# bioinformatics-centre/BayesTyper

Measured on AMD Instinct MI355X. Metric: variant-cluster Gibbs iterations/sec + k-mer matches/sec at 1/2/4/8 MI355X, higher is better.
Workload: dtype f64 log-probabilities over u8 k-mer counts (Gibbs); u64/u8 integer (k-mer matching)

## Files before the change

bayestyper_amd/csrc/bt_gibbs_simple.hpp:

```cpp
#pragma once
#include "bt_gibbs_tile.hpp"

namespace bt {

template <typename T>
struct LdsArr {
    T BT_LAS *p;
    __device__ inline T BT_LAS &operator[](uint32_t i) const { return p[i * LANES]; }
    __device__ inline LdsArr<T> operator+(uint32_t i) const { return LdsArr<T>{p + i * LANES}; }
};
template <typename T>
__device__ inline LdsArr<T> lds_arr(const Tile &t, int arr) {
    return LdsArr<T>{(T BT_LAS *)(bt_lds_raw + t.d->hoff[arr]) + t.lane};
}

struct Set2 {
    uint32_t n, e0, e1;
    __device__ inline void clear() { n = 0; }
    __device__ inline void insert(uint32_t e) {
        e1 = e0;
        e0 = e;
        ++n;
    }
    __device__ inline void erase(uint32_t e) {
// ... 232 lines not shown
        if (pv && pr > 255u) {
            log_collected_run(c, P, s, sd_key(pcode), pr, sc[SC_NSUB_U]);
            pr = 0;
            pv = 0;
        }
        blk[SB_WORDS * s + 2] = sd_code(dip[2 * s], dip[2 * s + 1]) | (pcode << SP_PDIP) | (wmax << SP_WMAX) | (pr << SP_PEND) | ((uint32_t)evn[s] << SP_EVN) | (pl << SP_PLOIDY) |
                                ((upd[s] ? 1u : 0u) << SP_UPD) | ((pv ? 1u : 0u) << SP_PVALID);
    }
    double p1 = 1.0;
    if (sc[SC_IS_SPARSE] && n_obs > 0) {
        TPtr<double> vec = c.simplex();
        const bool cached = d.scache_n && n_obs <= 2 * d.S && 1u <= d.scache_p;
        const uint32_t ci = cached ? (n_obs - 1) * d.scache_p : 0u;
        if (cached) vec = c.scache() + ci * d.scache_len;
        uint32_t len = cached ? (uint32_t)c.sclen()[ci] : 0u;
        if (len == 0) {
            len = simplex_prob_vector(c, P, vec, n_obs, 1u);
            if (cached) c.sclen()[ci] = len;
        }
        p1 = vec[0];
    }
    return p1;
}

__device__ static __noinline__ void simple_leave(Env env, uint32_t blk_off, double f0, double f1, uint32_t nzmask) {
    const Tile t = make_tile(env);
    const Vx c = make_vx(t, 0);
    const GParams BT_CAS &P = env_params(env);
    LdsArr<uint32_t> blk{(uint32_t BT_LAS *)(bt_lds_raw + blk_off) + t.lane};
    SPtrF<uint16_t, LANES> dip = c.dip(), pdip = c.pend_dip();
    SPtrF<uint32_t, LANES> pend = c.pend();
    SPtrF<uint8_t, LANES> pvalid = c.pend_valid(), upd = c.ksc_upd(), evn = c.evn();
    for (uint32_t s = 0; s < P.S; ++s) {
        const uint32_t pk = blk[SB_WORDS * s + 2];
        const uint32_t code = pk & 7u, pcode = (pk >> SP_PDIP) & 7u;
        dip[2 * s] = (uint16_t)sd_h1(code);
        dip[2 * s + 1] = (uint16_t)sd_h2(code);
        pdip[2 * s] = (uint16_t)sd_h1(pcode);
        pdip[2 * s + 1] = (uint16_t)sd_h2(pcode);
        pend[s] = (pk >> SP_PEND) & 255u;
        evn[s] = (uint8_t)((pk >> SP_EVN) & 255u);
        upd[s] = (uint8_t)((pk >> SP_UPD) & 1u);
        pvalid[s] = (uint8_t)((pk >> SP_PVALID) & 1u);
    }
    SPtrF<double, LANES> freq = c.freq(), logf = c.logf();
    SPtrF<uint8_t, LANES> nz = c.nz();
    freq[0] = f0;
    freq[1] = f1;
    nz[0] = (uint8_t)(nzmask & 1u);
    nz[1] = (uint8_t)((nzmask >> 1) & 1u);
    if (nzmask & 1u) logf[0] = bt_log(f0);
    if (nzmask & 2u) logf[1] = bt_log(f1);
}

__device__ static __noinline__ void simple_reweight(Env env, uint32_t blk_off) {
    const Tile t = make_tile(env);
    const Vx c = make_vx(t, 0);
    const GParams BT_CAS &P = env_params(env);
    simple_fill_unique(env);
    c.sc()[SC_UC_DIRTY] = 0;
    LdsArr<uint32_t> blk{(uint32_t BT_LAS *)(bt_lds_raw + blk_off) + t.lane};
    const Vx::UCPtr uc = c.ucache();
    const uint32_t Dcm = t.d->Dcm;
    for (uint32_t s = 0; s < P.S; ++s) {
        const uint32_t pk = blk[SB_WORDS * s + 2];
        const SimpleWeights w = simple_weights(uc, Dcm, s, (pk >> SP_PLOIDY) & 3u);
        blk[SB_WORDS * s] = __float_as_uint(w.ea);
        blk[SB_WORDS * s + 1] = __float_as_uint(w.eb);
        blk[SB_WORDS * s + 2] = (pk & ~(3u << SP_WMAX)) | (w.wmax << SP_WMAX);
    }
}
__device__ static __noinline__ void simple_noise_tally(Env env, uint32_t blk_off, const NoiseChainCtl *nc) {
    const Tile t = make_tile(env);
    const Vx c = make_vx(t, 0);
    const GParams BT_CAS &P = env_params(env);
    LdsArr<uint32_t> blk{(uint32_t BT_LAS *)(bt_lds_raw + blk_off) + t.lane};
    auto *bins = nc_bins(nc);
    const uint32_t nsu = c.sc()[SC_NSUB_U], Hm = t.d->Hm, S = P.S;
    const Vx::RPtr<uint8_t> sm = c.subm();
    TPtr<uint8_t> scn = c.subcnt(), sic = c.subic();
    for (uint32_t i = 0; i < nsu; i += 4) {
        uint8_t m0[4], m1[4], ic0[4], ic1[4];
#pragma unroll
        for (uint32_t r = 0; r < 4; ++r) {
            const uint32_t j = i + r < nsu ? i + r : nsu - 1u;
            m0[r] = sm[j * Hm];
            m1[r] = sm[j * Hm + 1];
            ic0[r] = sic[2 * j];
            ic1[r] = sic[2 * j + 1];
        }
        for (uint32_t s0 = 0; s0 < S; s0 += 4) {
            uint8_t cn[4][4];
#pragma unroll
            for (uint32_t w = 0; w < 4; ++w) {
                const uint32_t s = s0 + w < S ? s0 + w : S - 1u;
#pragma unroll
                for (uint32_t r = 0; r < 4; ++r) cn[w][r] = scn[(i + r < nsu ? i + r : nsu - 1u) * S + s];
            }
#pragma unroll
            for (uint32_t w = 0; w < 4; ++w) {
                const uint32_t s = s0 + w;
                if (s >= S) continue;
                const uint32_t code = blk[SB_WORDS * s + 2] & 7u, h1 = sd_h1(code), h2 = sd_h2(code);
                const bool g1 = P.gender[s] != 0;
#pragma unroll
                for (uint32_t r = 0; r < 4; ++r) {
                    uint8_t m = 0;
                    if (h1 != (uint32_t)NOHAP) m = (uint8_t)(m + (h1 ? m1[r] : m0[r]));
                    if (h2 != (uint32_t)NOHAP) m = (uint8_t)(m + (h2 ? m1[r] : m0[r]));
                    m = (uint8_t)(m + (g1 ? ic1[r] : ic0[r]));
                    if (i + r < nsu && m == 0) nc_tally(nc, bins, s, cn[w][r]);
                }
            }
        }
    }
    c.sc()[SC_UC_DIRTY] = 1;
}

__device__ inline void simple_sweeps(const Env &env, const Tile &t, const GParams BT_CAS &P, uint32_t n_burn, uint32_t n_collect, uint32_t *trace_counter, uint32_t *trace_buf,
                                     uint32_t trace_max, uint32_t tile, const NoiseChainCtl *nc = nullptr) {
    const uint32_t n_sweeps = n_burn + n_collect;
    const TileDesc BT_CAS &d = *t.d;
    const Vx c = make_vx(t, 0);
    const uint32_t S = P.S;
    const uint32_t blk_off = d.sblk;
    const double p_simplex1 = simple_enter(env, blk_off);
    LdsArr<uint32_t> blk{(uint32_t BT_LAS *)(bt_lds_raw + blk_off) + t.lane};
    SPtrF<uint32_t, LANES> sc = c.sc();
    const bool is_sparse = sc[SC_IS_SPARSE] != 0;
    Set2 zero{0, 0, 0}, plus{0, 0, 0};
    if (is_sparse) {
        zero = set2_load(c.zero_set());
        plus = set2_load(c.plus_set());
    }
    double fnd_saved = c.fnd_saved();
    uint32_t fnd_avail = sc[SC_FND_AVAIL];
    double f0, f1;
    uint32_t nzmask, obs0, obs1;
    {
        SPtrF<double, LANES> freq = c.freq();
        SPtrF<uint8_t, LANES> nz = c.nz();
        SPtrF<uint32_t, LANES> obs = c.obs();
        nzmask = (nz[0] ? 1u : 0u) | (nz[1] ? 2u : 0u);
        f0 = (nzmask & 1u) ? (double)freq[0] : 0.0;
        f1 = (nzmask & 2u) ? (double)freq[1] : 0.0;
        obs0 = obs[0];
        obs1 = obs[1];
    }
    typedef MtRingT<LdsArr<uint32_t>> Ring;
    const LdsArr<uint32_t> ring0 = lds_arr<uint32_t>(t, A_RING), ring1 = ring0 + (d.ring_cap[0] + MT_RING_HDR);
    Ring r0 = mt_ring_open_as(c.mt(0), ring0, d.ring_cap[0]), r1 = mt_ring_open_as(c.mt(1), ring1, d.ring_cap[1]);
    const double BT_GAS *a2tab = P.gamma_a2;
    const uint32_t a2n = P.gamma_n;

    const uint32_t sweep0 = nc ? nc->it_begin : 0u;
    for (uint32_t sweep = sweep0; sweep < n_sweeps; ++sweep) {
        const bool collect = sweep >= n_burn;
        if (nc && sweep > sweep0) {
            if (!nc_wait_table(nc, sweep)) break;
            if (nc->help_units) noise_help(env, nc);
            simple_reweight(env, blk_off);
        }
        bool tracing = false;
        TPtr<uint32_t> trace_row{(uint32_t BT_GAS *)trace_buf, 0u, 6u};
        if (trace_max) {
            uint32_t *cnt = &trace_counter[(size_t)tile * LANES + t.lane];
            const uint32_t n = *cnt;
            if (n < trace_max) {
                *cnt = n + 1;
                trace_row.off = (uint32_t)(d.trace_base + (size_t)n * d.nvm * S * LANES) + t.lane;
                tracing = true;
            }
        }
        PROF_DECL;
        {
            const uint32_t want = 2u * S < r0.cap - 3u ? 2u * S : r0.cap - 3u;
            if (bt_wave_any(r0.avail < want)) r0.topup();
            r1.topup();
        }
        PROF(11);
        const double ff00 = f0 * f0, ff01 = 2.0 * f0 * f1, ff11 = f1 * f1;
        const bool tiny = ((nzmask & 1u) && f0 < 1e-12) || ((nzmask & 2u) && f1 < 1e-12);
        for (uint32_t s = 0; s < S; ++s) {
            uint32_t pk = blk[SB_WORDS * s + 2];
            const float wa = __uint_as_float(blk[SB_WORDS * s]), wb = __uint_as_float(blk[SB_WORDS * s + 1]);
            const double u01 = rng_canonical(r0);
            const uint32_t pl = (pk >> SP_PLOIDY) & 3u, wmax = (pk >> SP_WMAX) & 3u, pcode = pk & 7u;
            uint32_t code = SD_NONE;
            if (pl != 0) {
                const double e0 = wmax == 0 ? 1.0 : (double)wa, e1 = wmax == 0 ? (double)wa : (wmax == 1 ? 1.0 : (double)wb), e2 = wmax == 2 ? 1.0 : (double)wb;
                const double w0 = (pl == 2 ? ff00 : f0) * e0, w1 = (pl == 2 ? ff01 : f1) * e1, w2 = pl == 2 ? ff11 * e2 : 0.0;
                const double c1 = w0 + w1, tot = c1 + w2, thr = u01 * tot, mg = 1e-5 * tot;
                const uint32_t pick = thr < w0 ? 0u : (thr < c1 ? 1u : 2u);
                const double lo = pick == 1 ? w0 : c1, hi = pick == 0 ? w0 : (pick == 1 ? c1 : tot);
                const bool safe = !tiny && tot > 1e-280 && hi - thr > mg && (pick == 0 || thr - lo > mg);
                code = pl == 2 ? pick : 3u + pick;
                if (!safe) {
                    PROF_CNT(19, 1);
                    code = simple_exact_code(env, s, pl, nzmask, f0, f1, u01);
                }
            }
            {
                const uint32_t h1 = sd_h1(code), h2 = sd_h2(code);
#pragma unroll
                for (uint32_t w = 0; w < 2; ++w) {
                    const uint32_t h = w ? h2 : h1;
                    if (h == (uint32_t)NOHAP) continue;
                    const uint32_t o = h ? obs1 : obs0;
                    if (is_sparse && o == 0) {
                        zero.erase(h);
                        plus.insert(h);
                    }
                    if (h) obs1 = o + 1;
                    else obs0 = o + 1;
                }
            }
            pk = (pk & ~7u) | code;
            if (code != pcode) pk |= 1u << SP_UPD;
            if (tracing) trace_row[s] = sd_key(code);
            if (collect) {
                const uint32_t pdc = (pk >> SP_PDIP) & 7u, run = (pk >> SP_PEND) & 255u;
                const bool pv = (pk >> SP_PVALID) & 1u;
                if (pv && pdc == code && run < 255u) pk += 1u << SP_PEND;
                else {
                    if (pv && run) {
                        uint32_t n = (pk >> SP_EVN) & 255u;
                        if (n == EV_CAP) {
                            simple_apply_full_log(env, s);
                            n = 0;
                        }
                        TPtr<uint32_t> lg = c.evlog(s);
                        lg[1 + 2 * n] = sd_key(pdc);
                        lg[2 + 2 * n] = run;
                        pk = (pk & ~(255u << SP_EVN)) | ((n + 1u) << SP_EVN);
                    }
                    pk = (pk & ~((7u << SP_PDIP) | (255u << SP_PEND))) | (code << SP_PDIP) | (1u << SP_PEND) | (1u << SP_PVALID);
                }
            }
            blk[SB_WORDS * s + 2] = pk;
        }
        PROF(2);
        const uint32_t n_obs = obs0 + obs1;
        if (n_obs > 0) {
            double saved = fnd_saved;
            uint32_t avail = fnd_avail;
            const NormalState nd{&saved, &avail};
            double g0 = 0, g1 = 0, norm = 0;
            bool sel0 = !is_sparse, sel1 = !is_sparse;
            uint32_t n_first = 2, n_steps = 2;
            Set2 order0 = plus;
            if (is_sparse) {
                const double u = rng_canonical(r1);
                n_first = plus.n;
                n_steps = plus.n + ((plus.n == 1 && !(u < p_simplex1)) ? 1u : 0u);
            }
            for (uint32_t i = 0; bt_wave_any(i < n_steps); ++i) {
                PROF_CNT(20, 1);
                if (i < n_steps) {
                    uint32_t e, o = 0;
                    if (!is_sparse) e = i;
                    else if (i < n_first) e = order0.at(i);
                    else {
                        const uint32_t pos = rng_uniform_int(r1, zero.n);
                        e = zero.at(pos);
                        zero.erase(e);
                        plus.insert(e);
                    }
                    if (i < n_first) o = e ? obs1 : obs0;
                    const uint32_t ai = o + 1u;
                    const double alpha = (double)ai, a1 = alpha - 1.0 / 3.0;
                    const double a2 = ai < a2n ? (double)a2tab[ai] : 1.0 / sqrt(9.0 * a1);
                    const double v = rng_gamma_v(r1, nd, a1, a2);
                    const double x = a1 * v * 1.0;
                    if (e) g1 = x, sel1 = true;
                    else g0 = x, sel0 = true;
                    norm += x;
                }
            }
            f0 = sel0 ? g0 / norm : 0.0;
            f1 = sel1 ? g1 / norm : 0.0;
            nzmask = (sel0 ? 1u : 0u) | (sel1 ? 2u : 0u);
            if (is_sparse) {
                const Set2 order = plus;
                plus.clear();
                for (uint32_t i = 0; i < 2; ++i)
                    if (i < order.n) zero.insert(order.at(i));
            }
            obs0 = obs1 = 0;
            fnd_saved = saved;
            fnd_avail = avail;
        }
        PROF(7);
        if (nc) {
            simple_noise_tally(env, blk_off, nc);
            if (!nc_iteration_end(nc, sweep)) break;
        }
    }
    mt_close(r0);
    mt_close(r1);
    if (is_sparse) {
        set2_store(c.zero_set(), zero);
        set2_store(c.plus_set(), plus);
    }
    c.fnd_saved() = fnd_saved;
    sc[SC_FND_AVAIL] = fnd_avail;
    sc[SC_HAP_COUNT] = obs0 + obs1;
// ... 11 lines not shown
```

bayestyper_amd/csrc/bt_gibbs_simple_kernel.hip:

```cpp
#define BT_SIMPLE_TU 1
#include "bt_gibbs_kernel.hpp"

namespace {
using namespace bt;
#ifndef GIBBS_SIMPLE_WAVES
#define GIBBS_SIMPLE_WAVES 3
#endif
__global__ __launch_bounds__(LANES, GIBBS_SIMPLE_WAVES) void gibbs_simple_kernel(const TileDesc *__restrict__ tiles, uint8_t *__restrict__ pool, const GParams *__restrict__ Pg,
                                                                                  int op, uint32_t arg0, uint32_t arg1, unsigned long long *__restrict__ hist, TraceCfg tr,
                                                                                  const uint32_t *__restrict__ tile_list) {
    gibbs_body<true>(tiles, pool, Pg, op, arg0, arg1, hist, tr, tile_list);
}
}

namespace bt {
hipError_t launch_gibbs_simple_kernel(unsigned grid, uint32_t lds, hipStream_t st, const TileDesc *tiles, uint8_t *pool, const GParams *P, int op, uint32_t a0, uint32_t a1,
                                      unsigned long long *hist, TraceCfg tr, const uint32_t *tile_list) {
    hipLaunchKernelGGL(gibbs_simple_kernel, dim3(grid), dim3(LANES), lds, st, tiles, pool, P, op, a0, a1, hist, tr, tile_list);
    return hipGetLastError();
}
#ifdef BT_PROF
hipError_t simple_prof_read(unsigned long long *h_out32, int reset) {
    hipError_t e = hipMemcpyFromSymbol(h_out32, HIP_SYMBOL(g_bt_prof), 32 * 8);
    if (e == hipSuccess && reset) {
        unsigned long long z[32] = {0};
        e = hipMemcpyToSymbol(HIP_SYMBOL(g_bt_prof), z, 32 * 8);
    }
    return e;
}
#endif
hipError_t prepare_gibbs_simple_kernel(int max_lds) {
    return hipFuncSetAttribute(reinterpret_cast<const void *>(gibbs_simple_kernel), hipFuncAttributeMaxDynamicSharedMemorySize, max_lds);
}
}
```

bayestyper_amd/csrc/bt_gibbs_tile.hpp:

```cpp
#pragma once
#include "bt_rng_device.hpp"

namespace bt {

constexpr unsigned LANES = 64;
constexpr uint16_t NOHAP = 0xFFFF;
constexpr double BT_LN2 = 0.693147180559945309417232121458176568;
constexpr double BT_DBL_EPS = 2.220446049250313080847263336181640625e-16;
#ifndef BT_LINEAR_DRAW_MIN
#define BT_LINEAR_DRAW_MIN 4u
#endif
#ifndef BT_UC_INVALIDATE_MIN
#define BT_UC_INVALIDATE_MIN 64u
#endif
#ifndef BT_EVAL_BLOCK
#define BT_EVAL_BLOCK 4u
#endif
constexpr uint32_t EVB = BT_EVAL_BLOCK;
#ifdef BT_SINGLE
constexpr bool kSingle = true;
#else
constexpr bool kSingle = false;
#endif
#ifdef BT_PACKED
// ... 1644 lines not shown
                        double fresh[EVB];
                        unique_log_prob_block(c, P, s, ha, hb, umiss, nsub_u, fresh);
#pragma unroll
                        for (uint32_t q = 0; q < EVB; ++q)
                            if (umiss[q]) uval[q] = fresh[q];
                    }
                }
#pragma unroll
                for (uint32_t q = 0; q < EVB; ++q) {
                    if (q < nb) {
                        double lp = 0;
                        if (!dipl) lp += la[q];
                        else if (ha[q] == hb[q]) lp += 2 * la[q];
                        else lp += BT_LN2 + la[q] + lb[q];
                        lp += uval[q];
                        if (multi) lp += mval[q];
                        lpmax = lp > lpmax ? lp : lpmax;
                        cum[base + q] = lp;
                    }
                }
                if (par) advance(EVB * (stride_blocks - 1u));
            }
            if (par) {
                const double own = lpmax;
                for (uint32_t m = 0; m < tsz; ++m) {
                    const double o = __shfl(own, (int)(tlane0 + m * cw));
                    lpmax = o > lpmax ? o : lpmax;
                }
                copies_sync();
            }
        };
        auto chain_pick = [&](double u01) -> uint32_t {
            if (total == 0) return 0u;
            double run = cum[0];
            for (uint32_t i = 1; i < total; ++i) {
                run = log_addition((double)cum[i], run);
                cum[i] = run;
            }
            const double u = bt_log(u01) + run;
            uint32_t lo = 0, hi = total;
            while (lo < hi) {
                const uint32_t mid = (lo + hi) >> 1;
                if (u < cum[mid]) hi = mid;
                else lo = mid + 1;
            }
            return lo < total ? lo : total - 1;
        };
        uint32_t pick = 0;
        for (bool exact = chain_only;; exact = true) {
            eval_candidates();
            PROF(2);
            if (exact) {
                if (total == 0) (void)bt_log(u01);
                pick = chain_pick(u01);
                PROF(28);
                break;
            }
            double acc = 0, thr = 0, off = 0;
            uint32_t s0 = 0, s1 = total;
            {
                const uint32_t ncp = tsz, L = (total + ncp - 1u) / ncp;
                const uint32_t i0 = tpart * L < total ? tpart * L : total, i1 = i0 + L < total ? i0 + L : total;
                double run = 0;
                for (uint32_t b0 = i0; b0 < i1; b0 += 8) {
                    double e[8];
#pragma unroll
                    for (uint32_t q = 0; q < 8; ++q) e[q] = b0 + q < i1 ? (double)cum[b0 + q] : 0.0;
#pragma unroll
                    for (uint32_t q = 0; q < 8; ++q)
                        if (b0 + q < i1) e[q] = bt_exp(e[q] - lpmax);
#pragma unroll
                    for (uint32_t q = 0; q < 8; ++q)
                        if (b0 + q < i1) {
                            run += e[q];
                            cum[b0 + q] = run;
                        }
                }
                for (uint32_t m = 0; m < ncp; ++m) acc += __shfl(run, (int)(tlane0 + m * cw));
                thr = u01 * acc;
                uint32_t seg = ncp;
                for (uint32_t m = 0; m < ncp; ++m) {
                    const double tseg = __shfl(run, (int)(tlane0 + m * cw));
                    if (seg == ncp) {
                        if (thr < off + tseg) seg = m;
                        else off += tseg;
                    }
                }
                if (tsz > 1u) copies_sync();
                s0 = seg * L < total ? seg * L : total;
                s1 = s0 + L < total ? s0 + L : total;
            }
            PROF(25);
            uint32_t lo = s0, hi = s1;
            while (lo < hi) {
                const uint32_t mid = (lo + hi) >> 1;
                if (thr < off + (double)cum[mid]) hi = mid;
                else lo = mid + 1;
            }
            const double amax = fabs(lpmax) > 1.0 ? fabs(lpmax) : 1.0;
            double margin = 64.0 * (double)total * amax * BT_DBL_EPS;
            margin = (margin > 1e-6 ? margin : 1e-6) * acc;
            const bool safe = lo < s1 && off + (double)cum[lo] - thr > margin && (lo == 0 || thr - (lo == s0 ? off : off + (double)cum[lo - 1]) > margin);
            PROF(26);
            if (safe) {
                pick = lo;
                break;
            }
            PROF_CNT(14, 1000000);
        }
        uint16_t h1 = NOHAP, h2 = NOHAP;
        if (ploidy == 2) {
            uint32_t a = 0, rem = pick;
            while (rem >= nnz - a) {
                rem -= nnz - a;
                ++a;
            }
            h1 = nzl[a];
            h2 = nzl[a + rem];
        } else if (ploidy == 1) {
            h1 = nzl[pick];
        }
        mine = (uint32_t)h1 | ((uint32_t)h2 << 16);
      }
      if (T > 1u) copies_sync();
      PROF(3);
      for (uint32_t j = 0; j < T && s0 + j < P.S; ++j) {
        const uint32_t ss = s0 + j;
        const uint32_t hh = T > 1u ? (uint32_t)__shfl((int)mine, (int)(gl + j * tsz * cw)) : mine;
        const uint16_t h1 = (uint16_t)(hh & 0xFFFFu), h2 = (uint16_t)(hh >> 16);
        const uint16_t p1 = dip[2 * ss], p2 = dip[2 * ss + 1];
        dip[2 * ss] = h1;
        dip[2 * ss + 1] = h2;
        if (!kSingle && c.d().nvm > 1u && (h1 != p1 || h2 != p2)) c.nver()[ss] += 1;
        hfd_increment(c, h1, is_sparse, hap_count);
        hfd_increment(c, h2, is_sparse, hap_count);
        PROF(4);
        update_multicluster_multiplicities(c, P, h1, h2, p1, p2, ss, nsub_m);
        PROF(5);
        if (tracing) trace_row[ss] = hh;
      }
    }
    mt_close(rng);
    sc[SC_HAP_COUNT] = hap_count;
#ifndef ABL_NOSTATS
    if (collect) update_allele_kmer_stats(env, vtx, nsub_u, nsub_m);
#endif
    PROF(6);
    sc[SC_USE_MULTI] = nsub_m != 0 ? 1u : 0u;
}

__device__ BT_SWEEPFN void rng_topup(Env env, uint32_t vtx) {
    const Vx c = make_vx(make_tile(env), vtx);
    MtRing a = c.rng(0), b = c.rng(1);
    a.topup();
    b.topup();
    mt_close(a);
    mt_close(b);
}

template <typename Q>
__device__ inline uint32_t simplex_prob_vector(const Vx &c, const GParams BT_CAS &P, Q out, uint32_t total_obs, uint32_t plus_size) {
    const uint32_t Hn = c.H;
    const double BT_GAS *lg = P.lgamma_int;
    const double sparsity = c.sparsity();
    const double lsp = bt_log(sparsity), l1sp = bt_log(1 - sparsity);
    double prob_z_log = plus_size * lsp + (Hn - plus_size) * l1sp;
    double prob_t_log = lg[plus_size] - lg[total_obs + plus_size];
    double prob_eq_z_log = 0.0 + prob_z_log + prob_t_log;
    double row_sum = prob_eq_z_log;
    uint32_t n = 0;
    out[n++] = row_sum;
    double prev = row_sum;
    for (uint32_t j = plus_size + 1; j < Hn + 1; ++j) {
        const double cardinal = lg[Hn - plus_size + 1] - (lg[j - plus_size + 1] + lg[Hn - j + 1]);
        prob_z_log = j * lsp + (Hn - j) * l1sp;
        prob_t_log = lg[j] - lg[total_obs + j];
        prob_eq_z_log = cardinal + prob_z_log + prob_t_log;
        row_sum += bt_log(1 + bt_exp(prob_eq_z_log - row_sum));
        out[n++] = row_sum;
        const double a = row_sum, b = prev;
        const double mn = a < b ? a : b;
        prev = row_sum;
        if (a == b || fabs(a - b) < fabs(mn) * BT_DBL_EPS * 100) break;
    }
    for (uint32_t i = 0; i < n; ++i) out[i] = bt_exp((double)out[i] - row_sum);
    return n;
}

template <class G>
__device__ inline double rng_gamma_count(G &rng, NormalState nd, const GParams BT_CAS &P, uint32_t count) {
    const uint32_t ai = count + 1u;
    const double a1 = (double)ai - 1.0 / 3.0;
    const double a2 = ai < P.gamma_n ? (double)P.gamma_a2[ai] : 1.0 / sqrt(9.0 * a1);
    return a1 * rng_gamma_v(rng, nd, a1, a2) * 1.0;
}

__device__ BT_SWEEPFN void sample_haplotype_frequencies(Env env, uint32_t vtx) {
    const Vx c = make_vx(make_tile(env), vtx);
    const GParams BT_CAS &P = env_params(env);
    const TileDesc BT_CAS &d = c.d();
    SPtrF<uint32_t, LANES> sc = c.sc();
    const uint32_t n_obs = sc[SC_HAP_COUNT];
    PROF_DECL;
    if (n_obs > 0) {
        MtRing rng = c.rng(1);
        const NormalState nd = c.fnd();
        SPtrF<uint32_t, LANES> obs = c.obs();
        SPtrF<double, LANES> freq = c.freq();
        SPtrF<uint8_t, LANES> nz = c.nz();
        if (!sc[SC_IS_SPARSE]) {
            double norm = 0;
            for (uint32_t h = 0; h < c.H; ++h) {
                const double f = rng_gamma_count(rng, nd, P, obs[h]);
                freq[h] = f;
                norm += f;
                obs[h] = 0;
            }
            SPtrF<double, LANES> logf = c.logf();
            for (uint32_t h = 0; h < c.H; ++h) {
                const double f = freq[h] / norm;
                freq[h] = f;
                logf[h] = bt_log(f);
            }
        } else {
            Vx::HSet plus = c.plus_set(), zero = c.zero_set();
            SPtrF<uint32_t, LANES> unext = c.unext();
            const uint32_t plus_size = uset_size(plus);
            uint32_t len;
            TPtr<double> vec = c.simplex();
            const bool cached = d.scache_n && n_obs <= 2 * d.S && plus_size <= d.scache_p;
            const uint32_t ci = cached ? (n_obs - 1) * d.scache_p + (plus_size - 1) : 0u;
            if (cached) vec = c.scache() + (uint32_t)ci * d.scache_len;
            constexpr uint32_t PRE = 4;
            const uint32_t pre = d.scache_len < PRE ? d.scache_len : PRE;
            double head[PRE];
#pragma unroll
            for (uint32_t q = 0; q < PRE; ++q) head[q] = (cached && q < pre) ? (double)vec[q] : 0.0;
            len = cached ? (uint32_t)c.sclen()[ci] : 0u;
            if (len == 0) {
                len = simplex_prob_vector(c, P, vec, n_obs, plus_size);
                if (cached) c.sclen()[ci] = len;
#pragma unroll
                for (uint32_t q = 0; q < PRE; ++q) head[q] = q < len ? (double)vec[q] : 0.0;
            }
            PROF(21);
            const double u = rng_canonical(rng);
            uint32_t ub = 0;
#pragma unroll
            for (uint32_t q = 0; q < PRE; ++q)
                if (ub == q && q < len && !(u < head[q])) ub = q + 1;
            if (ub == PRE)
                while (ub < len && !(u < vec[ub])) ++ub;
            const uint32_t simplex_size = ub + plus_size;
            double norm = 0;
            for (uint32_t e = uset_begin(plus); e != US_NONE; e = unext[e]) {
                const double f = rng_gamma_count(rng, nd, P, obs[e]);
                freq[e] = f;
                norm += f;
                nz[e] = 2;
            }
            PROF(22);
            while (uset_size(plus) < simplex_size) {
                const uint32_t pos = rng_uniform_int(rng, uset_size(zero));
                uint32_t e = uset_begin(zero);
                for (uint32_t i = 0; i < pos; ++i) e = unext[e];
                const double f = rng_gamma_count(rng, nd, P, 0u);
                freq[e] = f;
                norm += f;
                nz[e] = 2;
                uset_erase(zero, e);
                uset_insert(plus, e);
            }
            PROF(23);
            {
                uint32_t h = 0;
                for (; h + 8 <= c.H; h += 8) {
                    uint8_t m8[8];
#pragma unroll
                    for (int q = 0; q < 8; ++q) m8[q] = nz[h + q];
#pragma unroll
                    for (int q = 0; q < 8; ++q) {
                        if (m8[q] == 2) nz[h + q] = 1;
                        else {
                            freq[h + q] = 0;
                            nz[h + q] = 0;
                            obs[h + q] = 0;
                        }
                    }
                }
                for (; h < c.H; ++h) {
                    if (nz[h] == 2) nz[h] = 1;
                    else {
                        freq[h] = 0;
                        nz[h] = 0;
                        obs[h] = 0;
                    }
                }
            }
            SPtrF<uint16_t, LANES> nzl = c.nzlist();
            uint32_t np = 0;
            for (uint32_t e = uset_begin(plus); e != US_NONE; e = unext[e]) nzl[np++] = (uint16_t)e;
            uset_clear(plus);
            for (uint32_t i = 0; i < np; ++i) {
                const uint32_t e = nzl[i];
                const double f = freq[e] / norm;
                freq[e] = f;
                c.logf()[e] = bt_log(f);
                uset_insert(zero, e);
// ... 11 lines not shown
```

bayestyper_amd/csrc/bt_rng_device.hpp:

```cpp
#pragma once
#include <hip/hip_runtime.h>
#include <math.h>
#include <stdint.h>

namespace bt {

#define BT_HD __host__ __device__ inline
#if defined(BT_SIMPLE_TU) || defined(BT_SWEEP_INLINE)
#define BT_SWEEPFN inline
#else
#define BT_SWEEPFN static __noinline__
#endif
#define BT_NOINLINE static __noinline__

#if defined(__HIP_DEVICE_COMPILE__)
#define BT_MATH __host__ __device__ __noinline__
#ifdef BT_INLINE_MATH
#define BT_MATHI __host__ __device__ inline
#else
#define BT_MATHI BT_MATH
#endif
#else
#define BT_MATH __host__ __device__ inline
#define BT_MATHI BT_MATH
#endif
BT_MATHI double bt_log(double x) { return log(x); }
BT_MATHI double bt_exp(double x) { return exp(x); }
BT_MATH double bt_log1p(double x) { return log1p(x); }
BT_MATH double bt_pow(double x, double y) { return pow(x, y); }

#if defined(__HIP_DEVICE_COMPILE__)
#define BT_GAS __attribute__((address_space(1)))
#define BT_CAS __attribute__((address_space(4)))
#define BT_LAS __attribute__((address_space(3)))
#else
#define BT_GAS
#define BT_CAS
#define BT_LAS
#endif
template <typename T, unsigned STRIDE>
struct SPtr {
    T BT_GAS *base;
    uint32_t off;
    BT_HD T BT_GAS &operator[](uint32_t i) const { return base[off + i * STRIDE]; }
    BT_HD SPtr<T, STRIDE> operator+(uint32_t i) const { return SPtr<T, STRIDE>{base, off + i * STRIDE}; }
};
template <typename T>
BT_HD SPtr<T, 1> sptr1(T *p) { return SPtr<T, 1>{(T BT_GAS *)p, 0u}; }
template <typename T>
struct TPtr {
    T BT_GAS *base;
    uint32_t off;
    uint32_t sh;
    BT_HD T BT_GAS &operator[](uint32_t i) const { return base[off + (i << sh)]; }
    BT_HD TPtr<T> operator+(uint32_t i) const { return TPtr<T>{base, off + (i << sh), sh}; }
};
template <typename T, unsigned STRIDE>
struct SPtrF {
    T *base;
    uint32_t off;
    uint32_t sh = STRIDE == 64 ? 6u : 0u;
    BT_HD T &operator[](uint32_t i) const { return base[off + (i << sh)]; }
    BT_HD SPtrF<T, STRIDE> operator+(uint32_t i) const { return SPtrF<T, STRIDE>{base, off + (i << sh), sh}; }
};
#if defined(__HIP_DEVICE_COMPILE__)
template <typename T>
__device__ inline T *uniform_ptr(T *p) {
    const uint64_t v = (uint64_t)p;
    const uint32_t lo = __builtin_amdgcn_readfirstlane((uint32_t)v), hi = __builtin_amdgcn_readfirstlane((uint32_t)(v >> 32));
    return (T *)(((uint64_t)hi << 32) | lo);
}
#else
template <typename T>
__host__ __device__ inline T *uniform_ptr(T *p) { return p; }
#endif

constexpr unsigned MT_N = 624, MT_M = 397, MT_WORDS = 625;

BT_HD void mt_seed(uint32_t *st, uint32_t seed) {
    uint32_t x = seed;
    st[0] = x;
    for (unsigned i = 1; i < MT_N; ++i) {
        x = 1812433253u * (x ^ (x >> 30)) + i;
        st[i] = x;
    }
    st[MT_N] = 0;
}

BT_HD uint32_t mt_temper(uint32_t z) {
    z ^= (z >> 11);
    z ^= (z << 7) & 0x9d2c5680u;
    z ^= (z << 15) & 0xefc60000u;
    z ^= (z >> 18);
    return z;
}
BT_HD uint32_t mt_twist(uint32_t a, uint32_t b, uint32_t c) {
    const uint32_t y = (a & 0x80000000u) | (b & 0x7fffffffu);
    return c ^ (y >> 1) ^ ((y & 1u) ? 0x9908b0dfu : 0u);
}
BT_HD uint32_t mt_wrap(uint32_t i) { return i >= MT_N ? i - MT_N : i; }

struct Mt {
    uint32_t BT_GAS *st;
    uint32_t pos;
    BT_HD uint32_t next() {
        const uint32_t p = pos, p1 = mt_wrap(p + 1), pm = mt_wrap(p + MT_M);
        const uint32_t z = mt_twist(st[p], st[p1], st[pm]);
        st[p] = z;
        pos = p1;
        return mt_temper(z);
    }
    template <unsigned N>
    BT_HD void next_n(uint32_t (&out)[N]) {
        const uint32_t p = pos;
        uint32_t a[N + 1], c[N];
#pragma unroll
        for (uint32_t k = 0; k < N + 1; ++k) a[k] = st[mt_wrap(p + k)];
#pragma unroll
        for (uint32_t k = 0; k < N; ++k) c[k] = st[mt_wrap(mt_wrap(p + k) + MT_M)];
#pragma unroll
        for (uint32_t k = 0; k < N; ++k) {
            const uint32_t z = mt_twist(a[k], a[k + 1], c[k]);
            st[mt_wrap(p + k)] = z;
            out[k] = mt_temper(z);
        }
        pos = mt_wrap(p + N);
    }
};
BT_HD Mt mt_open(uint32_t *st) { return Mt{(uint32_t BT_GAS *)st, ((uint32_t BT_GAS *)st)[MT_N]}; }
BT_HD void mt_close(const Mt &m) { m.st[MT_N] = m.pos; }

constexpr unsigned MT_RING_HDR = 3;
constexpr unsigned MT_MIRROR = 4;
BT_HD void bt_sched_fence() {
#if defined(__HIP_DEVICE_COMPILE__)
    __builtin_amdgcn_sched_barrier(0);
#endif
}
BT_HD bool bt_wave_any(bool p) {
#if defined(__HIP_DEVICE_COMPILE__)
    return __builtin_amdgcn_ballot_w64(p) != 0;
#else
    return p;
#endif
}
#ifdef BT_DIAG_FAKE_MT
BT_HD uint32_t bt_fake_word(uint32_t x) {
    x ^= x >> 16;
    x *= 0x85ebca6bu;
    x ^= x >> 13;
    x *= 0xc2b2ae35u;
    x ^= x >> 16;
    return x;
}
#endif
#if !defined(BT_MT_CHUNK) && !defined(BT_MT_BLOCK)
#define BT_MT_BLOCK 1
#endif
constexpr unsigned MT_BUF = 640;
constexpr unsigned MT_AHEAD = 312;
constexpr uint32_t MT_F_CUR = 1u << 16, MT_F_READY = 1u << 17;
typedef uint32_t MtQuad __attribute__((ext_vector_type(4)));
typedef MtQuad MtQuadU __attribute__((aligned(4)));
#if defined(__HIP_DEVICE_COMPILE__)
__device__ inline void mt_twist_block(const uint32_t BT_GAS *old, uint32_t BT_GAS *nw) {
    const unsigned long long ex = __ballot(1);
    const uint32_t lane = threadIdx.x & 63u;
    const uint32_t rank = (uint32_t)__popcll(ex & ((1ull << lane) - 1ull)), n = (uint32_t)__popcll(ex);
    for (uint32_t q = rank; q < 57u; q += n) {
        const uint32_t va = 227u - 4u * q < 4u ? 227u - 4u * q : 4u;
        const uint32_t vc = q <= 42u ? (170u - 4u * q < 4u ? 170u - 4u * q : 4u) : 0u;
        const MtQuad a = *(const MtQuad BT_GAS *)(old + 4u * q);
        const uint32_t a4 = old[4u * q + 4u];
        const MtQuad b = *(const MtQuadU BT_GAS *)(old + 4u * q + 397u);
        const MtQuad c = *(const MtQuadU BT_GAS *)(old + 4u * q + 227u);
        const uint32_t c4 = old[4u * q + 231u];
        MtQuad d = {0u, 0u, 0u, 0u};
        uint32_t d4 = 0, o0 = 0, o1 = 0, o397 = 0;
        if (vc) {
            d = *(const MtQuadU BT_GAS *)(old + 4u * q + 454u);
            d4 = old[4u * q + 458u];
        }
        if (q == 42u) {
            o0 = old[0];
            o1 = old[1];
            o397 = old[397];
        }
        __builtin_amdgcn_sched_barrier(0);
        MtQuad za, zb, zc;
        za.x = mt_twist(a.x, a.y, b.x);
        za.y = mt_twist(a.y, a.z, b.y);
        za.z = mt_twist(a.z, a.w, b.z);
        za.w = mt_twist(a.w, a4, b.w);
        zb.x = mt_twist(c.x, c.y, za.x);
        zb.y = mt_twist(c.y, c.z, za.y);
        zb.z = mt_twist(c.z, c.w, za.z);
        zb.w = mt_twist(c.w, c4, za.w);
        const uint32_t new0 = mt_twist(o0, o1, o397);
        zc.x = mt_twist(d.x, d.y, zb.x);
        zc.y = mt_twist(d.y, q == 42u ? new0 : d.z, zb.y);
        zc.z = mt_twist(d.z, d.w, zb.z);
        zc.w = mt_twist(d.w, d4, zb.w);
        if (va == 4u) {
            *(MtQuad BT_GAS *)(nw + 4u * q) = za;
            *(MtQuadU BT_GAS *)(nw + 4u * q + 227u) = zb;
        } else {
            nw[4u * q] = za.x, nw[4u * q + 1u] = za.y, nw[4u * q + 2u] = za.z;
            nw[4u * q + 227u] = zb.x, nw[4u * q + 228u] = zb.y, nw[4u * q + 229u] = zb.z;
        }
        if (vc == 4u) *(MtQuadU BT_GAS *)(nw + 4u * q + 454u) = zc;
        else if (vc == 2u) nw[4u * q + 454u] = zc.x, nw[4u * q + 455u] = zc.y;
    }
    __builtin_amdgcn_fence(__ATOMIC_RELEASE, "workgroup");
    __builtin_amdgcn_wave_barrier();
    __builtin_amdgcn_fence(__ATOMIC_ACQUIRE, "workgroup");
}
__device__ static __noinline__ void mt_twist_for(bool want, uint32_t BT_GAS *st, uint32_t cur) {
    unsigned long long todo = __ballot(want);
    while (todo) {
        const int src = __builtin_ctzll(todo);
        const uint64_t p = (uint64_t)(uintptr_t)st;
        const uint32_t lo = (uint32_t)__builtin_amdgcn_readlane((int)(uint32_t)p, src), hi = (uint32_t)__builtin_amdgcn_readlane((int)(uint32_t)(p >> 32), src);
        const uint32_t c = (uint32_t)__builtin_amdgcn_readlane((int)cur, src);
        uint32_t BT_GAS *base = (uint32_t BT_GAS *)(uintptr_t)(((uint64_t)hi << 32) | lo);
        mt_twist_block(base + (c ? MT_BUF : 0u), base + (c ? 0u : MT_BUF));
        todo &= ~__ballot(want && (uint64_t)(uintptr_t)st == (((uint64_t)hi << 32) | lo));
    }
}
#endif
template <class RP>
struct MtRingT {
    uint32_t BT_GAS *st;
    RP ring;
    uint32_t cap;
    uint32_t pos, head, avail;
#ifdef BT_MT_BLOCK
    uint32_t flags = 0;
#endif
#ifdef BT_DIAG_FAKE_MT
    uint32_t fake_ctr = 0;
#endif
#if defined(BT_MT_BLOCK) && defined(__HIP_DEVICE_COMPILE__) && !defined(BT_DIAG_FAKE_MT)
    __device__ inline uint32_t BT_GAS *cur_buf() const { return st + ((flags & MT_F_CUR) ? MT_BUF : 0u); }
    __device__ inline void next_block(bool at_end) {
        mt_twist_for(at_end && !(flags & MT_F_READY), st, (flags & MT_F_CUR) ? 1u : 0u);
        if (at_end) {
            flags = (flags ^ MT_F_CUR) & ~MT_F_READY;
            pos = 0;
        }
    }
    __device__ inline void twist_ahead() {
        const bool want = pos >= MT_AHEAD && !(flags & MT_F_READY);
        if (bt_wave_any(want)) {
            mt_twist_for(want, st, (flags & MT_F_CUR) ? 1u : 0u);
            if (want) flags |= MT_F_READY;
        }
    }
    __device__ inline void chunk(bool go) {
        if (bt_wave_any(go && pos == MT_N)) next_block(go && pos == MT_N);
        if (go) {
            const MtQuad z = *(const MtQuad BT_GAS *)(cur_buf() + pos);
            const uint32_t w = (head + avail) & (cap - 1u);
            ring[w] = mt_temper(z.x);
            ring[w + 1u] = mt_temper(z.y);
            ring[w + 2u] = mt_temper(z.z);
            ring[w + 3u] = mt_temper(z.w);
            pos += 4u;
            avail += 4u;
        }
    }
    template <unsigned NB>
    __device__ inline void batch(uint32_t want) {
        if (bt_wave_any(avail < want && pos == MT_N)) next_block(avail < want && pos == MT_N);
        uint32_t nc = avail < want ? (want - avail + 3u) >> 2 : 0u;
        nc = nc < NB ? nc : NB;
        const uint32_t left = (MT_N - pos) >> 2;
        nc = nc < left ? nc : left;
        MtQuad z[NB];
        const uint32_t BT_GAS *b = cur_buf() + pos;
#pragma unroll
        for (unsigned j = 0; j < NB; ++j)
            if (j < nc) z[j] = *(const MtQuad BT_GAS *)(b + 4u * j);
        bt_sched_fence();
#pragma unroll
        for (unsigned j = 0; j < NB; ++j)
            if (j < nc) {
                const uint32_t w = (head + avail) & (cap - 1u);
                ring[w] = mt_temper(z[j].x);
                ring[w + 1u] = mt_temper(z[j].y);
                ring[w + 2u] = mt_temper(z[j].z);
                ring[w + 3u] = mt_temper(z[j].w);
                avail += 4u;
                pos += 4u;
            }
    }
    __device__ inline void fill_to(uint32_t want) {
        while (bt_wave_any(avail < want)) chunk(avail < want);
    }
    template <unsigned NB>
    __device__ inline void fill_batched(uint32_t want) {
        if (bt_wave_any(avail < want)) batch<NB>(want);
        fill_to(want);
    }
    __device__ inline void topup() {
        twist_ahead();
        fill_batched<4>(cap - 3u);
    }
#else
    BT_HD void chunk(bool go) {
#ifdef BT_DIAG_FAKE_MT
        if (go) {
            const uint32_t salt = (uint32_t)(uintptr_t)st * 2654435761u + fake_ctr;
            const uint32_t w = (head + avail) & (cap - 1u);
            for (uint32_t k = 0; k < 4u; ++k) ring[w + k] = bt_fake_word(salt + pos + k);
            fake_ctr += 0x9e3779b9u;
            pos = pos + 4u == MT_N ? 0u : pos + 4u;
            avail += 4u;
        }
        return;
#endif
        if (go) {
            const uint32_t p = pos, q = p + MT_M < MT_N ? p + MT_M : p + MT_M - MT_N;
            const MtQuad a = *(const MtQuad BT_GAS *)(st + p);
            const uint32_t a4 = st[p + 4u];
            const MtQuad b = *(const MtQuadU BT_GAS *)(st + q);
            bt_sched_fence();
            MtQuad z;
            z.x = mt_twist(a.x, a.y, b.x);
            z.y = mt_twist(a.y, a.z, b.y);
            z.z = mt_twist(a.z, a.w, b.z);
            z.w = mt_twist(a.w, a4, b.w);
            *(MtQuad BT_GAS *)(st + p) = z;
            if (p == 0) *(MtQuad BT_GAS *)(st + MT_N) = z;
            const uint32_t w = (head + avail) & (cap - 1u);
            ring[w] = mt_temper(z.x);
            ring[w + 1u] = mt_temper(z.y);
            ring[w + 2u] = mt_temper(z.z);
            ring[w + 3u] = mt_temper(z.w);
            pos = p + 4u == MT_N ? 0u : p + 4u;
            avail += 4u;
        }
    }
    template <unsigned NB>
    BT_HD void batch(uint32_t want) {
#ifdef BT_DIAG_FAKE_MT
        for (unsigned j = 0; j < NB; ++j) chunk(avail < want);
        return;
#endif
        uint32_t nc = avail < want ? (want - avail + 3u) >> 2 : 0u;
        nc = nc < NB ? nc : NB;
        MtQuad a[NB], b[NB];
        uint32_t a4[NB], pp[NB];
        uint32_t p = pos;
#pragma unroll
        for (unsigned j = 0; j < NB; ++j) {
            pp[j] = p;
            if (j < nc) {
                const uint32_t q = p + MT_M < MT_N ? p + MT_M : p + MT_M - MT_N;
                a[j] = *(const MtQuad BT_GAS *)(st + p);
                a4[j] = st[p + 4u];
                b[j] = *(const MtQuadU BT_GAS *)(st + q);
            }
            p = p + 4u == MT_N ? 0u : p + 4u;
        }
        bt_sched_fence();
#pragma unroll
        for (unsigned j = 0; j < NB; ++j)
            if (j < nc) {
                MtQuad z;
                z.x = mt_twist(a[j].x, a[j].y, b[j].x);
                z.y = mt_twist(a[j].y, a[j].z, b[j].y);
                z.z = mt_twist(a[j].z, a[j].w, b[j].z);
                z.w = mt_twist(a[j].w, a4[j], b[j].w);
                *(MtQuad BT_GAS *)(st + pp[j]) = z;
                if (pp[j] == 0) *(MtQuad BT_GAS *)(st + MT_N) = z;
                const uint32_t w = (head + avail) & (cap - 1u);
                ring[w] = mt_temper(z.x);
                ring[w + 1u] = mt_temper(z.y);
                ring[w + 2u] = mt_temper(z.z);
                ring[w + 3u] = mt_temper(z.w);
                avail += 4u;
                pos = pp[j] + 4u == MT_N ? 0u : pp[j] + 4u;
            }
    }
    BT_HD void fill_to(uint32_t want) {
        while (bt_wave_any(avail < want)) chunk(avail < want);
    }
    template <unsigned NB>
    BT_HD void fill_batched(uint32_t want) {
        if (bt_wave_any(avail < want)) batch<NB>(want);
        fill_to(want);
    }
    BT_HD void topup() { fill_batched<4>(cap - 3u); }
#endif
    BT_HD void need(uint32_t n) {
        if (avail < n) fill_to(cap - 3u < 16u ? cap - 3u : 16u);
    }
    BT_HD uint32_t next() {
        need(1);
        const uint32_t w = ring[head];
        head = (head + 1u) & (cap - 1u);
        avail -= 1u;
        return w;
    }
    template <unsigned N>
    BT_HD void next_n(uint32_t (&out)[N]) {
        need(N);
#pragma unroll
        for (uint32_t k = 0; k < N; ++k) out[k] = ring[(head + k) & (cap - 1u)];
        head = (head + N) & (cap - 1u);
        avail -= N;
    }
};
typedef MtRingT<SPtrF<uint32_t, 1>> MtRing;
template <class RP>
BT_HD MtRingT<RP> mt_ring_open_as(uint32_t *st, RP ring, uint32_t cap) {
    MtRingT<RP> m;
    m.st = (uint32_t BT_GAS *)st;
    m.ring = ring;
    m.cap = cap;
    m.pos = m.ring[cap];
    m.head = m.ring[cap + 1];
    m.avail = m.ring[cap + 2];
#ifdef BT_MT_BLOCK
    m.flags = m.pos & (MT_F_CUR | MT_F_READY);
    m.pos &= 0xFFFFu;
#endif
    return m;
}
template <class RP>
BT_HD MtRing mt_ring_open(uint32_t *st, RP ring, uint32_t cap) {
    MtRing m;
    m.st = (uint32_t BT_GAS *)st;
    m.ring = SPtrF<uint32_t, 1>{ring.base, ring.off, ring.sh};
    m.cap = cap;
    m.pos = m.ring[cap];
    m.head = m.ring[cap + 1];
    m.avail = m.ring[cap + 2];
#ifdef BT_MT_BLOCK
    m.flags = m.pos & (MT_F_CUR | MT_F_READY);
    m.pos &= 0xFFFFu;
#endif
    return m;
}
template <class RP>
BT_HD void mt_close(const MtRingT<RP> &m) {
#ifdef BT_MT_BLOCK
    m.ring[m.cap] = m.pos | m.flags;
#else
    m.ring[m.cap] = m.pos;
#endif
    m.ring[m.cap + 1] = m.head;
    m.ring[m.cap + 2] = m.avail;
}
template <class RP>
BT_HD void mt_ring_seed(uint32_t *st, RP ring, uint32_t cap, uint32_t seed) {
    mt_seed(st, seed);
    for (unsigned i = 0; i < MT_MIRROR; ++i) st[MT_N + i] = st[i];
#ifdef BT_MT_BLOCK
    ring[cap] = MT_N;
#else
    ring[cap] = 0;
#endif
    ring[cap + 1] = 0;
    ring[cap + 2] = 0;
}

template <class G>
BT_HD uint32_t mt_next(G &m) { return m.next(); }

template <class G>
BT_HD double rng_canonical(G &m) {
    uint32_t w[2];
    m.template next_n<2>(w);
    double sum = (double)w[0];
    sum += (double)w[1] * 4294967296.0;
    double ret = sum / 18446744073709551616.0;
    if (ret >= 1.0) ret = 0.99999999999999988897769753748434595763683319091796875;
    return ret;
}

template <class G>
BT_HD void rng_canonical2(G &m, double &first, double &second) {
    uint32_t w[4];
    m.template next_n<4>(w);
    const double top = 0.99999999999999988897769753748434595763683319091796875;
    double s0 = (double)w[0];
    s0 += (double)w[1] * 4294967296.0;
    first = s0 / 18446744073709551616.0;
    if (first >= 1.0) first = top;
    double s1 = (double)w[2];
    s1 += (double)w[3] * 4294967296.0;
    second = s1 / 18446744073709551616.0;
    if (second >= 1.0) second = top;
}

template <class G>
BT_HD uint32_t rng_uniform_int(G &st, uint32_t range) {
    uint64_t product = (uint64_t)mt_next(st) * (uint64_t)range;
    uint32_t low = (uint32_t)product;
    if (low < range) {
        uint32_t threshold = (0u - range) % range;
        while (low < threshold) {
            product = (uint64_t)mt_next(st) * (uint64_t)range;
            low = (uint32_t)product;
        }
    }
    return (uint32_t)(product >> 32);
}

template <class G>
BT_HD bool rng_bernoulli(G &st, double p) { return rng_canonical(st) < p; }

template <class G, typename Arr>
BT_HD void rng_shuffle_u32(G &st, Arr a, uint32_t n) {
    if (n == 0) return;
    const uint64_t urngrange = 0xFFFFFFFFull;
    if (urngrange / n >= n) {
        uint32_t i = 1;
        if ((n % 2u) == 0) {
            uint32_t j = rng_uniform_int(st, 2);
            uint32_t t = a[i]; a[i] = a[j]; a[j] = t;
            ++i;
        }
        while (i != n) {
            const uint32_t swap_range = i + 1;
            const uint32_t b1 = swap_range + 1;
            uint32_t x = rng_uniform_int(st, swap_range * b1);
            uint32_t p0 = x / b1, p1 = x % b1;
            uint32_t t = a[i]; a[i] = a[p0]; a[p0] = t;
            ++i;
            t = a[i]; a[i] = a[p1]; a[p1] = t;
            ++i;
        }
        return;
    }
    for (uint32_t i = 1; i < n; ++i) {
        uint32_t j = rng_uniform_int(st, i + 1);
        uint32_t t = a[i]; a[i] = a[j]; a[j] = t;
    }
}

struct NormalState {
    double *saved;
    uint32_t *available;
};

template <class G>
BT_HD double rng_normal(G &st, NormalState nd) {
// ... 195 lines not shown
```

Baseline: 1.211 billion.

## Software-pipeline MT twist across rings and split RNG top-up into issue/commit

Restructures the Mersenne Twister block twist so that one wave processes all requesting rings in a single loop, with the loads for the next quad issued before the current quad's stores. This overlaps global memory latency with the twist arithmetic. RNG top-up is split into prepare, issue and commit phases so the loads for both rings are in flight together before tempering. An urgency threshold defers twist-ahead in the simple kernel, and BT_NO_NOISE_CHAIN is defined for the simple kernel TU. The risks are extra register pressure from the pending quads and deferred twists that could stall later draws.

```diff
diff --git a/bayestyper_amd/csrc/bt_gibbs_simple.hpp b/bayestyper_amd/csrc/bt_gibbs_simple.hpp
--- a/bayestyper_amd/csrc/bt_gibbs_simple.hpp
+++ b/bayestyper_amd/csrc/bt_gibbs_simple.hpp
@@ -408,6 +408,10 @@
     Ring r0 = mt_ring_open_as(c.mt(0), ring0, d.ring_cap[0]), r1 = mt_ring_open_as(c.mt(1), ring1, d.ring_cap[1]);
     const double BT_GAS *a2tab = P.gamma_a2;
     const uint32_t a2n = P.gamma_n;
+#ifdef BT_MT_BLOCK
+    r0.urgent = 2u * S <= 64u ? MT_URGENT_SIMPLE : MT_AHEAD;
+    r1.urgent = MT_URGENT_SIMPLE;
+#endif
 
     const uint32_t sweep0 = nc ? nc->it_begin : 0u;
     for (uint32_t sweep = sweep0; sweep < n_sweeps; ++sweep) {
diff --git a/bayestyper_amd/csrc/bt_gibbs_simple_kernel.hip b/bayestyper_amd/csrc/bt_gibbs_simple_kernel.hip
--- a/bayestyper_amd/csrc/bt_gibbs_simple_kernel.hip
+++ b/bayestyper_amd/csrc/bt_gibbs_simple_kernel.hip
@@ -1,4 +1,5 @@
 #define BT_SIMPLE_TU 1
+#define BT_NO_NOISE_CHAIN 1
 #include "bt_gibbs_kernel.hpp"
 
 namespace {
diff --git a/bayestyper_amd/csrc/bt_gibbs_tile.hpp b/bayestyper_amd/csrc/bt_gibbs_tile.hpp
--- a/bayestyper_amd/csrc/bt_gibbs_tile.hpp
+++ b/bayestyper_amd/csrc/bt_gibbs_tile.hpp
@@ -1820,8 +1820,15 @@
 __device__ BT_SWEEPFN void rng_topup(Env env, uint32_t vtx) {
     const Vx c = make_vx(make_tile(env), vtx);
     MtRing a = c.rng(0), b = c.rng(1);
-    a.topup();
-    b.topup();
+    a.topup_prepare();
+    b.topup_prepare();
+    a.topup_issue();
+    b.topup_issue();
+    bt_sched_fence();
+    a.topup_commit();
+    b.topup_commit();
+    a.fill_to(a.cap - 3u);
+    b.fill_to(b.cap - 3u);
     mt_close(a);
     mt_close(b);
 }
diff --git a/bayestyper_amd/csrc/bt_rng_device.hpp b/bayestyper_amd/csrc/bt_rng_device.hpp
--- a/bayestyper_amd/csrc/bt_rng_device.hpp
+++ b/bayestyper_amd/csrc/bt_rng_device.hpp
@@ -159,73 +159,115 @@
 #endif
 constexpr unsigned MT_BUF = 640;
 constexpr unsigned MT_AHEAD = 312;
+constexpr unsigned MT_PEND = 4;
+constexpr unsigned MT_URGENT_SIMPLE = MT_N - 128;
 constexpr uint32_t MT_F_CUR = 1u << 16, MT_F_READY = 1u << 17;
 typedef uint32_t MtQuad __attribute__((ext_vector_type(4)));
 typedef MtQuad MtQuadU __attribute__((aligned(4)));
 #if defined(__HIP_DEVICE_COMPILE__)
-__device__ inline void mt_twist_block(const uint32_t BT_GAS *old, uint32_t BT_GAS *nw) {
+struct MtTwistIn {
+    MtQuad a, b, c, d;
+    uint32_t a4, c4, d4, o0, o1, o397;
+};
+struct MtTwistOut {
+    MtQuad za, zb, zc;
+};
+__device__ inline void mt_twist_load(const uint32_t BT_GAS *old, uint32_t q, MtTwistIn &in) {
+    in.a = *(const MtQuad BT_GAS *)(old + 4u * q);
+    in.a4 = old[4u * q + 4u];
+    in.b = *(const MtQuadU BT_GAS *)(old + 4u * q + 397u);
+    in.c = *(const MtQuadU BT_GAS *)(old + 4u * q + 227u);
+    in.c4 = old[4u * q + 231u];
+    in.d = MtQuad{0u, 0u, 0u, 0u};
+    in.d4 = 0, in.o0 = 0, in.o1 = 0, in.o397 = 0;
+    if (q <= 42u) {
+        in.d = *(const MtQuadU BT_GAS *)(old + 4u * q + 454u);
+        in.d4 = old[4u * q + 458u];
+    }
+    if (q == 42u) {
+        in.o0 = old[0];
+        in.o1 = old[1];
+        in.o397 = old[397];
+    }
+}
+__device__ inline void mt_twist_compute(uint32_t q, const MtTwistIn &in, MtTwistOut &z) {
+    z.za.x = mt_twist(in.a.x, in.a.y, in.b.x);
+    z.za.y = mt_twist(in.a.y, in.a.z, in.b.y);
+    z.za.z = mt_twist(in.a.z, in.a.w, in.b.z);
+    z.za.w = mt_twist(in.a.w, in.a4, in.b.w);
+    z.zb.x = mt_twist(in.c.x, in.c.y, z.za.x);
+    z.zb.y = mt_twist(in.c.y, in.c.z, z.za.y);
+    z.zb.z = mt_twist(in.c.z, in.c.w, z.za.z);
+    z.zb.w = mt_twist(in.c.w, in.c4, z.za.w);
+    const uint32_t new0 = mt_twist(in.o0, in.o1, in.o397);
+    z.zc.x = mt_twist(in.d.x, in.d.y, z.zb.x);
+    z.zc.y = mt_twist(in.d.y, q == 42u ? new0 : in.d.z, z.zb.y);
+    z.zc.z = mt_twist(in.d.z, in.d.w, z.zb.z);
+    z.zc.w = mt_twist(in.d.w, in.d4, z.zb.w);
+}
+__device__ inline void mt_twist_store(uint32_t BT_GAS *nw, uint32_t q, const MtTwistOut &z) {
+    const uint32_t va = 227u - 4u * q < 4u ? 227u - 4u * q : 4u;
+    const uint32_t vc = q <= 42u ? (170u - 4u * q < 4u ? 170u - 4u * q : 4u) : 0u;
+    if (va == 4u) {
+        *(MtQuad BT_GAS *)(nw + 4u * q) = z.za;
+        *(MtQuadU BT_GAS *)(nw + 4u * q + 227u) = z.zb;
+    } else {
+        nw[4u * q] = z.za.x, nw[4u * q + 1u] = z.za.y, nw[4u * q + 2u] = z.za.z;
+        nw[4u * q + 227u] = z.zb.x, nw[4u * q + 228u] = z.zb.y, nw[4u * q + 229u] = z.zb.z;
+    }
+    if (vc == 4u) *(MtQuadU BT_GAS *)(nw + 4u * q + 454u) = z.zc;
+    else if (vc == 2u) nw[4u * q + 454u] = z.zc.x, nw[4u * q + 455u] = z.zc.y;
+}
+__device__ static __noinline__ void mt_twist_for(bool want, uint32_t BT_GAS *st, uint32_t cur) {
+    unsigned long long todo = __ballot(want);
+    if (!todo) return;
     const unsigned long long ex = __ballot(1);
     const uint32_t lane = threadIdx.x & 63u;
     const uint32_t rank = (uint32_t)__popcll(ex & ((1ull << lane) - 1ull)), n = (uint32_t)__popcll(ex);
-    for (uint32_t q = rank; q < 57u; q += n) {
-        const uint32_t va = 227u - 4u * q < 4u ? 227u - 4u * q : 4u;
-        const uint32_t vc = q <= 42u ? (170u - 4u * q < 4u ? 170u - 4u * q : 4u) : 0u;
-        const MtQuad a = *(const MtQuad BT_GAS *)(old + 4u * q);
-        const uint32_t a4 = old[4u * q + 4u];
-        const MtQuad b = *(const MtQuadU BT_GAS *)(old + 4u * q + 397u);
-        const MtQuad c = *(const MtQuadU BT_GAS *)(old + 4u * q + 227u);
-        const uint32_t c4 = old[4u * q + 231u];
-        MtQuad d = {0u, 0u, 0u, 0u};
-        uint32_t d4 = 0, o0 = 0, o1 = 0, o397 = 0;
-        if (vc) {
-            d = *(const MtQuadU BT_GAS *)(old + 4u * q + 454u);
-            d4 = old[4u * q + 458u];
-        }
-        if (q == 42u) {
-            o0 = old[0];
-            o1 = old[1];
-            o397 = old[397];
-        }
+    const uint32_t rounds = (57u + n - 1u) / n;
+    const uint64_t mine = (uint64_t)(uintptr_t)st;
+    const uint32_t BT_GAS *s_old = nullptr;
+    uint32_t BT_GAS *s_new = nullptr;
+    uint32_t round = rounds;
+    auto next_quad = [&](const uint32_t BT_GAS *&old, uint32_t BT_GAS *&nw, uint32_t &q) -> bool {
+        if (round == rounds) {
+            if (!todo) return false;
+            const int src = __builtin_ctzll(todo);
+            const uint32_t lo = (uint32_t)__builtin_amdgcn_readlane((int)(uint32_t)mine, src), hi = (uint32_t)__builtin_amdgcn_readlane((int)(uint32_t)(mine >> 32), src);
+            const uint32_t c = (uint32_t)__builtin_amdgcn_readlane((int)cur, src);
+            uint32_t BT_GAS *base = (uint32_t BT_GAS *)(uintptr_t)(((uint64_t)hi << 32) | lo);
+            s_old = base + (c ? MT_BUF : 0u);
+            s_new = base + (c ? 0u : MT_BUF);
+            todo &= ~__ballot(want && mine == (((uint64_t)hi << 32) | lo));
+            round = 0;
+        }
+        old = s_old;
+        nw = s_new;
+        q = rank + round * n;
+        ++round;
+        return true;
+    };
+    const uint32_t BT_GAS *old;
+    uint32_t BT_GAS *nw;
+    uint32_t q;
+    bool more = next_quad(old, nw, q);
+    MtTwistIn in{};
+    if (q < 57u) mt_twist_load(old, q, in);
+    while (more) {
         __builtin_amdgcn_sched_barrier(0);
-        MtQuad za, zb, zc;
-        za.x = mt_twist(a.x, a.y, b.x);
-        za.y = mt_twist(a.y, a.z, b.y);
-        za.z = mt_twist(a.z, a.w, b.z);
-        za.w = mt_twist(a.w, a4, b.w);
-        zb.x = mt_twist(c.x, c.y, za.x);
-        zb.y = mt_twist(c.y, c.z, za.y);
-        zb.z = mt_twist(c.z, c.w, za.z);
-        zb.w = mt_twist(c.w, c4, za.w);
-        const uint32_t new0 = mt_twist(o0, o1, o397);
-        zc.x = mt_twist(d.x, d.y, zb.x);
-        zc.y = mt_twist(d.y, q == 42u ? new0 : d.z, zb.y);
-        zc.z = mt_twist(d.z, d.w, zb.z);
-        zc.w = mt_twist(d.w, d4, zb.w);
-        if (va == 4u) {
-            *(MtQuad BT_GAS *)(nw + 4u * q) = za;
-            *(MtQuadU BT_GAS *)(nw + 4u * q + 227u) = zb;
-        } else {
-            nw[4u * q] = za.x, nw[4u * q + 1u] = za.y, nw[4u * q + 2u] = za.z;
-            nw[4u * q + 227u] = zb.x, nw[4u * q + 228u] = zb.y, nw[4u * q + 229u] = zb.z;
-        }
-        if (vc == 4u) *(MtQuadU BT_GAS *)(nw + 4u * q + 454u) = zc;
-        else if (vc == 2u) nw[4u * q + 454u] = zc.x, nw[4u * q + 455u] = zc.y;
+        MtTwistOut z;
+        mt_twist_compute(q, in, z);
+        asm volatile("" : "+v"(z.za), "+v"(z.zb), "+v"(z.zc) : : "memory");
+        uint32_t BT_GAS *const nw_now = nw;
+        const uint32_t q_now = q;
+        more = next_quad(old, nw, q);
+        if (more && q < 57u) mt_twist_load(old, q, in);
+        __builtin_amdgcn_sched_barrier(0);
+        if (q_now < 57u) mt_twist_store(nw_now, q_now, z);
     }
     __builtin_amdgcn_fence(__ATOMIC_RELEASE, "workgroup");
     __builtin_amdgcn_wave_barrier();
     __builtin_amdgcn_fence(__ATOMIC_ACQUIRE, "workgroup");
-}
-__device__ static __noinline__ void mt_twist_for(bool want, uint32_t BT_GAS *st, uint32_t cur) {
-    unsigned long long todo = __ballot(want);
-    while (todo) {
-        const int src = __builtin_ctzll(todo);
-        const uint64_t p = (uint64_t)(uintptr_t)st;
-        const uint32_t lo = (uint32_t)__builtin_amdgcn_readlane((int)(uint32_t)p, src), hi = (uint32_t)__builtin_amdgcn_readlane((int)(uint32_t)(p >> 32), src);
-        const uint32_t c = (uint32_t)__builtin_amdgcn_readlane((int)cur, src);
-        uint32_t BT_GAS *base = (uint32_t BT_GAS *)(uintptr_t)(((uint64_t)hi << 32) | lo);
-        mt_twist_block(base + (c ? MT_BUF : 0u), base + (c ? 0u : MT_BUF));
-        todo &= ~__ballot(want && (uint64_t)(uintptr_t)st == (((uint64_t)hi << 32) | lo));
-    }
 }
 #endif
 template <class RP>
@@ -236,6 +278,9 @@
     uint32_t pos, head, avail;
 #ifdef BT_MT_BLOCK
     uint32_t flags = 0;
+    uint32_t urgent = MT_AHEAD;
+    uint32_t npend = 0;
+    MtQuad pend[MT_PEND];
 #endif
 #ifdef BT_DIAG_FAKE_MT
     uint32_t fake_ctr = 0;
@@ -251,7 +296,7 @@
     }
     __device__ inline void twist_ahead() {
         const bool want = pos >= MT_AHEAD && !(flags & MT_F_READY);
-        if (bt_wave_any(want)) {
+        if (bt_wave_any(want && pos >= urgent)) {
             mt_twist_for(want, st, (flags & MT_F_CUR) ? 1u : 0u);
             if (want) flags |= MT_F_READY;
         }
@@ -305,6 +350,37 @@
     __device__ inline void topup() {
         twist_ahead();
         fill_batched<4>(cap - 3u);
+    }
+    __device__ inline void topup_prepare() {
+        twist_ahead();
+        const bool flip = avail < cap - 3u && pos == MT_N;
+        if (bt_wave_any(flip)) next_block(flip);
+    }
+    __device__ inline void topup_issue() {
+        const uint32_t want = cap - 3u;
+        uint32_t nc = avail < want ? (want - avail + 3u) >> 2 : 0u;
+        nc = nc < MT_PEND ? nc : MT_PEND;
+        const uint32_t left = (MT_N - pos) >> 2;
+        nc = nc < left ? nc : left;
+        const uint32_t BT_GAS *b = cur_buf() + pos;
+#pragma unroll
+        for (unsigned j = 0; j < MT_PEND; ++j)
+            if (j < nc) pend[j] = *(const MtQuad BT_GAS *)(b + 4u * j);
+        npend = nc;
+    }
+    __device__ inline void topup_commit() {
+#pragma unroll
+        for (unsigned j = 0; j < MT_PEND; ++j)
+            if (j < npend) {
+                const uint32_t w = (head + avail) & (cap - 1u);
+                ring[w] = mt_temper(pend[j].x);
+                ring[w + 1u] = mt_temper(pend[j].y);
+                ring[w + 2u] = mt_temper(pend[j].z);
+                ring[w + 3u] = mt_temper(pend[j].w);
+                avail += 4u;
+                pos += 4u;
+            }
+        npend = 0;
     }
 #else
     BT_HD void chunk(bool go) {
@@ -392,9 +468,18 @@
         fill_to(want);
     }
     BT_HD void topup() { fill_batched<4>(cap - 3u); }
+    BT_HD void topup_prepare() {}
+    BT_HD void topup_issue() { topup(); }
+    BT_HD void topup_commit() {}
 #endif
     BT_HD void need(uint32_t n) {
-        if (avail < n) fill_to(cap - 3u < 16u ? cap - 3u : 16u);
+        if (avail < n) {
+#if defined(BT_MT_BLOCK) && defined(__HIP_DEVICE_COMPILE__) && !defined(BT_DIAG_FAKE_MT)
+            if (npend) topup_commit();
+            if (avail >= n) return;
+#endif
+            fill_to(cap - 3u < 16u ? cap - 3u : 16u);
+        }
     }
     BT_HD uint32_t next() {
         need(1);
```

Measured after the change: 1.219 billion (median of 5 runs). About the same (+0.6%).
